# RayforceDB/rayforce

Measured on AMD Instinct MI355X. Metric: rows/s on filter→group-by→sum, 1e9-row i64/f64; % HBM roofline at 1/2/4/8 GPU, higher is better.
Workload: dtype f64

## Files before the change

rayforce_amd/csrc/rfx_group_plane.hip:

```cpp
#include "rfx_part_common.hpp"
#include <stdlib.h>

#define PL_T 1024
#define PL_WAVES (PL_T / RFX_WAVE)
#define PL_WROWS 512
#define PL_BLOCK_ROWS (1 << 18)
#define PL_DELTA_BITS 18
#define PL_SLOT_BITS 14
#define PL_QCAP 320
#define PL_QFLUSH 24
#define PL_SPIN_LIMIT (1u << 14)
#define PL_MAX_NV 3
#ifndef PL_META64_PLAIN
#define PL_META64_PLAIN 1
#endif

struct PlaneArgs {
    int nblk;
    int nv;
    unsigned pmask;
    i64 block_rows;
    unsigned c0;
    u64 *vals[PL_MAX_NV];
    unsigned *meta;
    unsigned *cnt;
    unsigned *ctl;
};
struct PlSh {
    unsigned dead, _pad[3];
    i64 red[3][PL_WAVES];
};
template <int PBITS, int VGL, bool HK>
__host__ __device__ constexpr int pl_parts() { return (HK && PBITS == 8 && VGL == 4) ? 192 : (1 << PBITS); }
template <int NV, int PBITS, int VGL, bool HK = false>
__host__ __device__ constexpr size_t pl_lds_bytes() {
    return (size_t)pl_parts<PBITS, VGL, HK>() * ((size_t)(2 << VGL) * (NV * 8 + 4) + 8 + 4) + (size_t)PL_WAVES * PL_QCAP * 4 + sizeof(PlSh) + 64;
}
typedef u64 pl_v2 __attribute__((ext_vector_type(2)));
typedef unsigned pl_m2 __attribute__((ext_vector_type(2)));
#define PL_LD(ptr) __hip_atomic_load((ptr), __ATOMIC_RELAXED, __HIP_MEMORY_SCOPE_WORKGROUP)
#define PL_ST(ptr, v) __hip_atomic_store((ptr), (v), __ATOMIC_RELAXED, __HIP_MEMORY_SCOPE_WORKGROUP)

template <int NC, int NP, int NV, int PBITS, int VGL, bool HK = false>
__global__ __launch_bounds__(PL_T) void k_plane_scatter(const Plan P, const PlaneArgs A) {
    constexpr int PARTS = pl_parts<PBITS, VGL, HK>();
    constexpr bool P192 = PARTS != (1 << PBITS);
    constexpr unsigned VG = 1u << VGL, RING = 2u << VGL;
    constexpr bool KVI = HK && NV == 2 && PBITS == 8 && VGL == 3;
    constexpr unsigned LPD = VG / 2;
    extern __shared__ __attribute__((aligned(16))) unsigned char pl_smem[];
    u64 *vring = (u64 *)pl_smem;
    unsigned *mring = (unsigned *)(vring + (size_t)NV * PARTS * RING);
    unsigned *words = mring + (size_t)PARTS * RING;
    unsigned *tail = words + PARTS * 2;
    unsigned *fq = tail + PARTS;
    PlSh &L = *(PlSh *)(fq + PL_WAVES * PL_QCAP);
    PredSet<NP> S;
    predset_load<NP>(P, S);
    const int tid = threadIdx.x, lane = tid & 63, wv = tid >> 6;
    unsigned *myq = fq + wv * PL_QCAP;
    const i64 r0 = (i64)blockIdx.x * A.block_rows;
    const i64 r1 = (r0 + A.block_rows < P.nrows) ? r0 + A.block_rows : P.nrows;
    const u64 region = ((u64)blockIdx.x * (u64)PARTS) * A.c0;
    for (int i = tid; i < PARTS; i += PL_T) {
        tail[i] = 0;
        words[2 * i] = 0;
        words[2 * i + 1] = 0;
    }
    if (tid == 0) L.dead = 0;
    __syncthreads();
    i64 mn = RFX_INF_I64_D, mx = RFX_NULL_I64_D;
    unsigned nsel = 0;
    int qn = 0;

    auto flush_queue = [&]() __attribute__((always_inline)) {
        asm volatile("" ::: "memory");
        for (int i0 = 0; i0 < qn; i0 += 64 / (int)LPD) {
            const int idx = i0 + (lane / (int)LPD);
            if (idx < qn) {
                const unsigned d = myq[idx];
                const unsigned p = d & 0xFFu, gi = (d >> 8) & 0x3FFFFFu, pl = d >> 30, sub = lane & (LPD - 1u);
                if (pl < 3) {
                    const pl_v2 x = *(const pl_v2 *)(vring + ((size_t)pl * PARTS + p) * RING + (gi & 1u) * VG + sub * 2);
                    if constexpr (KVI) {
                        __builtin_nontemporal_store(x, (pl_v2 *)(A.vals[0] + 2 * (region + (u64)p * A.c0 + (u64)gi * VG) + (u64)pl * VG + sub * 2));
                    } else {
                        u64 *dst = (NV == 1 ? A.vals[0] : (pl == 0 ? A.vals[0] : (pl == 1 ? A.vals[1] : A.vals[2])));
                        __builtin_nontemporal_store(x, (pl_v2 *)(dst + region + (u64)p * A.c0 + (u64)gi * VG + sub * 2));
                    }
                } else if (sub < LPD / 2) {
                    const pl_v2 x = *(const pl_v2 *)(mring + (size_t)p * RING + (gi & 1u) * VG + sub * 4);
                    if constexpr (KVI || (VGL == 4 && PL_META64_PLAIN)) *(pl_v2 *)(A.meta + region + (u64)p * A.c0 + (u64)gi * VG + sub * 4) = x;
                    else __builtin_nontemporal_store(x, (pl_v2 *)(A.meta + region + (u64)p * A.c0 + (u64)gi * VG + sub * 4));
                }
            }
        }
        asm volatile("" ::: "memory");
        for (int i = lane; i < qn; i += 64) {
            const unsigned d = myq[i];
            if ((d >> 30) == 3u) atomicAdd(&words[2 * (d & 0xFFu) + ((d >> 8) & 1u)], 256u - VG);
        }
        qn = 0;
    };

    auto place = [&](const bool on, const u64 key, const u64 (&val)[NV], const unsigned delta) __attribute__((always_inline)) {
        const u64 kh = HK ? rfx_hash_index_u64(RFX_U64_HASH_SEED, key) : key;
        const unsigned p = P192 ? (unsigned)(((kh >> 32) * (u64)PARTS) >> 32) : (HK ? (unsigned)(kh >> (64 - PBITS)) : ((unsigned)key & (unsigned)(PARTS - 1)));
        unsigned seq = 0;
        if (on) {
            const i64 k = (i64)key;
            mn = k < mn ? k : mn;
            mx = k > mx ? k : mx;
            seq = atomicAdd(&tail[p], 1u);
            if (seq >= A.c0) PL_ST(&L.dead, 1u);
        }
        const unsigned g = seq >> VGL;
        unsigned *w = &words[2 * p + (g & 1u)];
        bool todo = on && seq < A.c0;
        for (unsigned it = 0;; it++) {
            bool ready = false;
            if (todo) ready = (PL_LD(w) >> 8) == (g >> 1);
            bool comp = false;
            if (ready) {
                const unsigned at = p * RING + (seq & (RING - 1u));
#pragma unroll
                for (int j = 0; j < NV; j++) vring[(size_t)j * PARTS * RING + at] = val[j];
                mring[at] = ((unsigned)(P192 ? (kh >> 18) : (HK ? (kh >> (64 - PBITS - PL_SLOT_BITS)) : (key >> PBITS))) & ((1u << PL_SLOT_BITS) - 1u)) | (delta << PL_SLOT_BITS);
                asm volatile("" ::: "memory");
                comp = (atomicAdd(w, 1u) & 0xFFu) == VG - 1u;
                todo = false;
            }
            const u64 cb = __ballot(comp);
            if (cb) {
                if (comp) {
                    const unsigned at = (unsigned)qn + (unsigned)(NV + 1) * __builtin_amdgcn_mbcnt_hi((unsigned)(cb >> 32), __builtin_amdgcn_mbcnt_lo((unsigned)cb, 0u));
#pragma unroll
                    for (int j = 0; j < NV; j++) myq[at + j] = p | (g << 8) | ((unsigned)j << 30);
                    myq[at + NV] = p | (g << 8) | (3u << 30);
                }
                qn += (NV + 1) * __popcll(cb);
            }
            if (!__any(todo)) break;
            flush_queue();
            if (PL_LD(&L.dead) || it > PL_SPIN_LIMIT) {
                PL_ST(&L.dead, 1u);
                break;
            }
            if (it) __builtin_amdgcn_s_sleep(4);
        }
        if (qn >= PL_QFLUSH) flush_queue();
    };

    bool alive = true;
    auto step = [&](const u64 (&v)[NC][8], const unsigned m, const i64 sbase) __attribute__((always_inline)) {
        const unsigned dbase = (unsigned)(sbase - r0);
        const unsigned valid = m;
        if constexpr (NP == 0) {
            nsel += (unsigned)__popc(valid);
#pragma unroll
            for (int e = 0; e < 8; e++) {
                u64 val[NV];
#pragma unroll
                for (int j = 0; j < NV; j++) val[j] = v[1 + j][e];
                place((valid >> e) & 1u, v[0][e], val, dbase + (unsigned)((e >> 1) * 128 + (e & 1)));
            }
        } else {
            unsigned rem = m;
            nsel += (unsigned)__popc(rem);
            u64 t[1 + NV][8];
#pragma unroll
            for (int c = 0; c < 1 + NV; c++) {
#pragma unroll
                for (int q = 0; q < 8; q++) {
                    t[c][q] = v[c][q];
                    if constexpr (NV > 1) asm volatile("" : "+v"(t[c][q]));
                }
            }
            while (__any(rem != 0u)) {
                const bool on = rem != 0u;
                const unsigned e = (unsigned)__builtin_ctz(rem | 0x100u);
                rem &= rem - 1u;
                u64 key = t[0][0], val[NV];
#pragma unroll
                for (int j = 0; j < NV; j++) val[j] = t[1 + j][0];
#pragma unroll
                for (int q = 1; q < 8; q++) {
                    const bool is = e == (unsigned)q;
                    key = is ? t[0][q] : key;
#pragma unroll
                    for (int j = 0; j < NV; j++) val[j] = is ? t[1 + j][q] : val[j];
                }
                place(on, key, val, dbase + (e >> 1) * 128u + (e & 1u));
            }
        }
        flush_queue();
        if (PL_LD(&L.dead)) alive = false;
    };

    const i64 nsteps = (r1 - r0 + PL_WROWS - 1) / PL_WROWS;
    const i64 nfull = (r1 - r0) / PL_WROWS;
    {
        u64 va[NC][8];
        for (i64 s = wv; s < nfull && alive; s += PL_WAVES) {
            const i64 base = r0 + s * PL_WROWS + lane * 2;
            if constexpr (NP == 0) {
#pragma unroll
                for (int c = 0; c < NC; c++) {
#pragma unroll
                    for (int j = 0; j < 4; j++) {
                        const u64x2 t = rfx_ld2(P.cols[c] + base + j * 128);
                        va[c][2 * j] = t.x;
                        va[c][2 * j + 1] = t.y;
                    }
                }
                step(va, 0xffu, base);
            } else {
#pragma unroll
                for (int c = 0; c < NC; c++) {
                    if ((A.pmask >> c) & 1u) {
#pragma unroll
                        for (int j = 0; j < 4; j++) {
                            const u64x2 t = rfx_ld2(P.cols[c] + base + j * 128);
                            va[c][2 * j] = t.x;
                            va[c][2 * j + 1] = t.y;
                        }
                    } else {
#pragma unroll
                        for (int e = 0; e < 8; e++) va[c][e] = 0;
                    }
                }
                const unsigned m = eval_preds<NC, 8, NP>(S, va, 0xffu);
#pragma unroll
                for (int c = 0; c < NC; c++) {
                    if (!((A.pmask >> c) & 1u)) {
#pragma unroll
                        for (int j = 0; j < 4; j++) {
                            if ((m >> (2 * j)) & 3u) {
                                const u64x2 t = rfx_ld2(P.cols[c] + base + j * 128);
                                va[c][2 * j] = t.x;
                                va[c][2 * j + 1] = t.y;
                            }
                        }
                    }
                }
                step(va, m, base);
            }
        }
    }
    if (nfull < nsteps && (nfull % PL_WAVES) == wv && alive) {
        u64 va[NC][8];
        const i64 base = r0 + nfull * PL_WROWS + lane * 2;
        unsigned valid = 0;
#pragma unroll
        for (int e = 0; e < 8; e++) {
            const i64 row = base + (e >> 1) * 128 + (e & 1);
            const bool in = row < r1;
            valid |= (unsigned)in << e;
#pragma unroll
            for (int c = 0; c < NC; c++) va[c][e] = in ? P.cols[c][row] : 0ULL;
        }
        step(va, (NP == 0) ? valid : eval_preds<NC, 8, NP>(S, va, valid), base);
    }
    __syncthreads();
    if (L.dead) {
        if (tid == 0) atomicExch(&A.ctl[1], 1u);
        return;
    }
    for (int i = tid; i < PARTS * (NV + 1) * (int)LPD; i += PL_T) {
        const unsigned sub = (unsigned)i & (LPD - 1u), p = ((unsigned)i / LPD) % (unsigned)PARTS, pl = ((unsigned)i / LPD) / (unsigned)PARTS;
        const unsigned t = tail[p];
        if (!(t & (VG - 1u))) continue;
        const unsigned gi = t >> VGL;
        if (pl < (unsigned)NV) {
            const pl_v2 x = *(const pl_v2 *)(vring + ((size_t)pl * PARTS + p) * RING + (gi & 1u) * VG + sub * 2);
            if constexpr (KVI) {
                *(pl_v2 *)(A.vals[0] + 2 * (region + (u64)p * A.c0 + (u64)gi * VG) + (u64)pl * VG + sub * 2) = x;
            } else {
                u64 *dst = (NV == 1 ? A.vals[0] : (pl == 0 ? A.vals[0] : (pl == 1 ? A.vals[1] : A.vals[2])));
                *(pl_v2 *)(dst + region + (u64)p * A.c0 + (u64)gi * VG + sub * 2) = x;
            }
        } else if (sub < LPD / 2) {
            const pl_v2 x = *(const pl_v2 *)(mring + (size_t)p * RING + (gi & 1u) * VG + sub * 4);
            *(pl_v2 *)(A.meta + region + (u64)p * A.c0 + (u64)gi * VG + sub * 4) = x;
        }
    }
    for (int i = tid; i < PARTS; i += PL_T) A.cnt[(size_t)blockIdx.x * PARTS + i] = tail[i];
    i64 sel = (i64)nsel;
    for (int s2 = 32; s2 >= 1; s2 >>= 1) {
        const i64 omn = (i64)rfx_shfl_xor_u64((u64)mn, s2), omx = (i64)rfx_shfl_xor_u64((u64)mx, s2);
        mn = omn < mn ? omn : mn;
        mx = omx > mx ? omx : mx;
        sel += (i64)rfx_shfl_xor_u64((u64)sel, s2);
    }
    if (lane == 0) {
        L.red[0][wv] = mn;
        L.red[1][wv] = mx;
        L.red[2][wv] = sel;
    }
    __syncthreads();
    if (tid == 0) {
        for (int w2 = 1; w2 < PL_WAVES; w2++) {
            mn = L.red[0][w2] < mn ? L.red[0][w2] : mn;
            mx = L.red[1][w2] > mx ? L.red[1][w2] : mx;
            sel += L.red[2][w2];
        }
        unsigned long long *g = (unsigned long long *)A.ctl + 8;
        if (sel > 0) {
            atomicMax(&g[0], ~((unsigned long long)mn ^ 0x8000000000000000ULL));
            atomicMax(&g[1], (unsigned long long)mx ^ 0x8000000000000000ULL);
            atomicAdd(&g[2], (unsigned long long)sel);
        }
    }
}

struct PlaneAggArgs {
    i64 kmin, range;
    i64 local;
    int split;
    int excl;
    int first_read;
    int nblk, pbits;
    int agg_pl[RFX_MAX_AGGS];
    i64 block_rows;
    unsigned c0;
    const u64 *vals[PL_MAX_NV];
    const unsigned *meta;
    const unsigned *cnt;
    u64 *first;
    u64 *acc[RFX_MAX_AGGS];
    u64 *cntt[RFX_MAX_AGGS];
};
#define PL_FIRST_NONE 0xFFFFFFFFu

template <int THREADS, int NVL, bool FAST>
__global__ __launch_bounds__(THREADS) void k_plane_aggregate(const Plan P, const PlaneAggArgs A) {
    extern __shared__ __attribute__((aligned(16))) u64 pl_agg_smem[];
    const int tid = threadIdx.x;
    const int p = blockIdx.x / A.split, s = blockIdx.x % A.split;
    const i64 local = A.local;
    int kind[RFX_MAX_AGGS], f64[RFX_MAX_AGGS], skip[RFX_MAX_AGGS], cnt_of[RFX_MAX_AGGS], apl[RFX_MAX_AGGS];
    int ncnt = 0;
#pragma unroll
    for (int a = 0; a < RFX_MAX_AGGS; a++) {
        kind[a] = (a < P.nagg) ? P.aggs[a].kind : -1;
        f64[a] = (a < P.nagg) ? P.aggs[a].f64 : 0;
        skip[a] = (a < P.nagg) ? P.aggs[a].skipnull : 0;
        apl[a] = (a < P.nagg) ? A.agg_pl[a] : -1;
        cnt_of[a] = -1;
        if (kind[a] >= 0 && agg_has_cnt(kind[a], f64[a])) cnt_of[a] = ncnt++;
    }
    u64 *accs = pl_agg_smem;
    unsigned *first = (unsigned *)(accs + (i64)P.nagg * local);
    unsigned *cnts = first + local;
    for (i64 i = tid; i < local; i += THREADS) first[i] = PL_FIRST_NONE;
#pragma unroll
    for (int a = 0; a < RFX_MAX_AGGS; a++) {
        if (kind[a] < 0) continue;
        const u64 id = acc_identity(kind[a], f64[a]);
        for (i64 i = tid; i < local; i += THREADS) accs[(i64)a * local + i] = id;
        if (cnt_of[a] >= 0) {
            for (i64 i = tid; i < local; i += THREADS) cnts[(i64)cnt_of[a] * local + i] = 0u;
        }
    }
    __syncthreads();
    const unsigned shift = (unsigned)(((i64)p - A.kmin) >> A.pbits);
    auto apply = [&](unsigned mm, i64 rbase, const u64 (&x)[NVL]) __attribute__((always_inline)) {
        const unsigned mask = (1u << PL_SLOT_BITS) - 1u;
        const unsigned slot = ((mm & mask) + shift) & mask;
        if ((i64)slot >= local) return;
        const unsigned row = (unsigned)(rbase + (i64)(mm >> PL_SLOT_BITS));
        if (A.first_read) {
            if (row < first[slot]) atomicMin(&first[slot], row);
        } else __hip_atomic_fetch_min(&first[slot], row, __ATOMIC_RELAXED, __HIP_MEMORY_SCOPE_WORKGROUP);
        if constexpr (FAST) {
            unsafeAtomicAdd((double *)&accs[slot], rfx_as_f64(x[0]));
            return;
        }
#pragma unroll
        for (int a = 0; a < RFX_MAX_AGGS; a++) {
            if (kind[a] < 0) continue;
            u64 xv = 0;
#pragma unroll
            for (int j = 0; j < NVL; j++)
                if (apl[a] == j) xv = x[j];
            group_apply(&accs[(i64)a * local + slot], cnt_of[a] >= 0 ? &cnts[(i64)cnt_of[a] * local + slot] : (unsigned *)0, kind[a], f64[a], xv, skip[a]);
        }
    };
    const int lane = tid & 63;
    constexpr int NW = THREADS / 64;
    const int Q = A.split * NW;
    struct Batch {
        pl_v2 val[NVL][2];
        pl_m2 m[2];
        unsigned n, i0;
        int b;
    };
    auto load = [&](bool live, int b, unsigned i0, unsigned n, Batch &B) __attribute__((always_inline)) {
        B.b = live ? b : 0;
        B.i0 = live ? i0 : 0u;
        B.n = live ? n : 0u;
        const u64 base = (((u64)B.b << A.pbits) + (u64)p) * A.c0;
#pragma unroll
        for (int k = 0; k < 2; k++) {
            unsigned i = B.i0 + ((unsigned)k * 64u + (unsigned)lane) * 2u;
            i = i < A.c0 - 2u ? i : A.c0 - 2u;
#pragma unroll
            for (int j = 0; j < NVL; j++) B.val[j][k] = __builtin_nontemporal_load((const pl_v2 *)(A.vals[j] + base + i));
            B.m[k] = __builtin_nontemporal_load((const pl_m2 *)(A.meta + base + i));
        }
    };
    auto consume = [&](const Batch &B) __attribute__((always_inline)) {
        const i64 rbase = (i64)B.b * A.block_rows;
#pragma unroll
        for (int k = 0; k < 2; k++) {
            const unsigned i = B.i0 + ((unsigned)k * 64u + (unsigned)lane) * 2u;
            if (i < B.n) {
                u64 x[NVL];
#pragma unroll
                for (int j = 0; j < NVL; j++) x[j] = B.val[j][k].x;
                apply(B.m[k].x, rbase, x);
                if (i + 1 < B.n) {
#pragma unroll
                    for (int j = 0; j < NVL; j++) x[j] = B.val[j][k].y;
                    apply(B.m[k].y, rbase, x);
                }
            }
        }
    };
    const int q = __builtin_amdgcn_readfirstlane(s * NW + (tid >> 6));
    const int nreg = q < A.nblk ? (A.nblk - q + Q - 1) / Q : 0;
    unsigned *wcnt = cnts + (i64)ncnt * local + (tid >> 6) * 64;
    int r = -1;
    int b = q;
    unsigned i0 = 0, n = 0;
    auto advance = [&]() __attribute__((always_inline)) {
        for (;;) {
            if (r >= 0 && i0 < n) return true;
            r++;
            if (r >= nreg) return false;
            if ((r & 63) == 0) {
                const int r0 = r + lane;
                wcnt[lane] = (r0 < nreg) ? A.cnt[((size_t)(q + r0 * Q) << A.pbits) + p] : 0u;
            }
            n = (unsigned)__builtin_amdgcn_readfirstlane((int)wcnt[r & 63]);
            b = q + r * Q;
            i0 = 0;
        }
    };
    Batch B0, B1;
    bool h0 = advance();
    load(h0, b, i0, n, B0);
    i0 += 256u;
    while (h0) {
        const bool h1 = advance();
        load(h1, b, i0, n, B1);
        i0 += 256u;
        consume(B0);
        if (!h1) break;
        h0 = advance();
        load(h0, b, i0, n, B0);
        i0 += 256u;
        consume(B1);
    }
    __syncthreads();
    for (i64 i = tid; i < local; i += THREADS) {
        const unsigned f = first[i];
        if (f == PL_FIRST_NONE) continue;
        const i64 g = (i << A.pbits) | (i64)(((u64)p - (u64)A.kmin) & (u64)((1 << A.pbits) - 1));
        if (g >= A.range) continue;
        const u64 fr = (u64)P.row0 + (u64)f;
        if (A.excl) {
            if (fr < A.first[g]) A.first[g] = fr;
#pragma unroll
            for (int a = 0; a < RFX_MAX_AGGS; a++) {
                if (kind[a] < 0) continue;
                const bool hc = cnt_of[a] >= 0;
                group_merge_cell_plain(&A.acc[a][g], hc ? &A.cntt[a][g] : (u64 *)0, kind[a], f64[a], accs[(i64)a * local + i], hc ? (u64)cnts[(i64)cnt_of[a] * local + i] : 0ULL);
            }
            continue;
        }
        if (fr < A.first[g]) atomicMin((unsigned long long *)&A.first[g], (unsigned long long)fr);
#pragma unroll
        for (int a = 0; a < RFX_MAX_AGGS; a++) {
            if (kind[a] < 0) continue;
            const bool hc = cnt_of[a] >= 0;
            group_merge_cell(&A.acc[a][g], hc ? &A.cntt[a][g] : (u64 *)0, kind[a], f64[a], accs[(i64)a * local + i], hc ? (u64)cnts[(i64)cnt_of[a] * local + i] : 0ULL);
        }
    }
}

int rfx_chunk_reserve(rfx_ctx *c, size_t bytes);
static size_t pl_al256(size_t x) { return (x + 255) & ~(size_t)255; }

static void plane_layout(rfx_ctx *c, int nblk, int pbits, unsigned c0, int nv, PlaneArgs *A, size_t *total, int parts = 0) {
    const size_t regions = parts ? (size_t)nblk * (size_t)parts : (size_t)nblk << pbits;
    const size_t o_cnt = 256;
    const size_t o_meta = o_cnt + pl_al256(regions * 4), o_val = o_meta + pl_al256(regions * c0 * 4);
    const size_t plane = pl_al256(regions * c0 * 8);
    if (total) *total = o_val + plane * nv;
    char *w = (char *)c->d_chunk;
    A->nblk = nblk;
    A->nv = nv;
    A->c0 = c0;
    A->ctl = (unsigned *)w;
    A->cnt = (unsigned *)(w + o_cnt);
    A->meta = (unsigned *)(w + o_meta);
    for (int j = 0; j < nv; j++) A->vals[j] = (u64 *)(w + o_val + plane * j);
}

template <int NC, int NP, int NV, int PBITS, int VGL, bool HK = false>
static int launch_plane_scatter_inst(rfx_ctx *c, const Plan &P, const PlaneArgs &A) {
    constexpr size_t lds = pl_lds_bytes<NV, PBITS, VGL, HK>();
    static_assert(lds <= 160 * 1024, "rings beyond a CU's LDS");
    static unsigned long long attr_set = 0;
    if (!((attr_set >> (c->device & 63)) & 1ull)) {
        RFX_HIP_CHECK(hipFuncSetAttribute((const void *)k_plane_scatter<NC, NP, NV, PBITS, VGL, HK>, hipFuncAttributeMaxDynamicSharedMemorySize, (int)lds));
        __atomic_fetch_or(&attr_set, 1ull << (c->device & 63), __ATOMIC_RELAXED);
    }
    hipLaunchKernelGGL((k_plane_scatter<NC, NP, NV, PBITS, VGL, HK>), dim3(A.nblk), dim3(PL_T), lds, c->stream, P, A);
    return RFX_OK;
}
template <int NC, int NV, int PBITS, int VGL, bool HK = false>
static int launch_plane_scatter_np(rfx_ctx *c, const Plan &P, const PlaneArgs &A) {
    if (P.npred == 0) return launch_plane_scatter_inst<NC, 0, NV, PBITS, VGL, HK>(c, P, A);
    if (P.npred == 1) return launch_plane_scatter_inst<NC, 1, NV, PBITS, VGL, HK>(c, P, A);
    if (P.npred <= 3) return launch_plane_scatter_inst<NC, 3, NV, PBITS, VGL, HK>(c, P, A);
    return launch_plane_scatter_inst<NC, RFX_MAX_PREDS, NV, PBITS, VGL, HK>(c, P, A);
}
static int launch_plane_scatter(rfx_ctx *c, const Plan &P, const PlaneArgs &A, int pbits) {
    const int extra = P.ncols - 1 - A.nv;
    if (extra < 0 || extra > 2) return RFX_ESTATE;
    if (A.nv == 1) {
        if (pbits == 7) return extra == 0 ? launch_plane_scatter_np<2, 1, 7, 5>(c, P, A) : (extra == 1 ? launch_plane_scatter_np<3, 1, 7, 5>(c, P, A) : launch_plane_scatter_np<4, 1, 7, 5>(c, P, A));
        return extra == 0 ? launch_plane_scatter_np<2, 1, 8, 4>(c, P, A) : (extra == 1 ? launch_plane_scatter_np<3, 1, 8, 4>(c, P, A) : launch_plane_scatter_np<4, 1, 8, 4>(c, P, A));
    }
    if (pbits != 7 || extra > 1) return RFX_ESTATE;
    if (A.nv == 2) return extra == 0 ? launch_plane_scatter_np<3, 2, 7, 4>(c, P, A) : launch_plane_scatter_np<4, 2, 7, 4>(c, P, A);
    return extra == 0 ? launch_plane_scatter_np<4, 3, 7, 4>(c, P, A) : launch_plane_scatter_np<5, 3, 7, 4>(c, P, A);
}

static int plane_value_cols(const Plan &P, int *vcol, int *agg_plane) {
    int nv = 0;
    for (int a = 0; a < P.nagg; a++) {
        const PlanAgg &ag = P.aggs[a];
        agg_plane[a] = -1;
        if (ag.kind == RFX_AGG_COUNT || ag.kind == RFX_AGG_FIRST || ag.col < 0) continue;
        if (ag.col >= RFX_XCOL) return -1;
        int j = 0;
        for (; j < nv; j++)
            if (vcol[j] == ag.col) break;
        if (j == nv) {
            if (nv >= PL_MAX_NV) return -1;
            vcol[nv++] = ag.col;
        }
        agg_plane[a] = j;
    }
    return nv;
}
static size_t plane_agg_lds(const Plan &P, int a0, int a1, i64 local) {
    size_t cells8 = 0, cells4 = 1;
    for (int a = a0; a < a1; a++) {
        cells8++;
        if (agg_has_cnt(P.aggs[a].kind, P.aggs[a].f64)) cells4++;
    }
    return (size_t)local * (cells8 * 8 + cells4 * 4) + 16 * 64 * 4 + 64;
}
#define PL_AGG_LDS_MAX (150 * 1024)
static bool plane_agg_fits(const Plan &P, i64 local) {
    for (int a = 0; a < P.nagg; a++)
        if (plane_agg_lds(P, a, a + 1, local) > PL_AGG_LDS_MAX) return false;
    return P.nagg >= 1;
}

struct PlaneState {
    int valid, npred, logic, nblk, pbits, nv;
    unsigned c0;
    const void *key;
    const void *val[PL_MAX_NV];
    i64 nrows;
    i64 seen;
    u64 sig[RFX_MAX_PREDS][6];
};
static PlaneState *plane_state(rfx_ctx *c) {
    if (!c->ext_p[2]) c->ext_p[2] = calloc(1, sizeof(PlaneState));
    return (PlaneState *)c->ext_p[2];
}
void rfx_plane_invalidate(rfx_ctx *c) {
    if (c->ext_p[2]) ((PlaneState *)c->ext_p[2])->valid = 0;
}
void rfx_plane_release(rfx_ctx *c) {
    free(c->ext_p[2]);
    c->ext_p[2] = NULL;
}
static void plane_pred_sig(const Plan &P, u64 (*sig)[6]) {
    for (int i = 0; i < P.npred; i++) {
        const PlanPred &q = P.preds[i];
        sig[i][0] = (u64)(uintptr_t)P.cols[q.col];
        sig[i][1] = q.rhs_col >= 0 ? (u64)(uintptr_t)P.cols[q.rhs_col] : 0;
        sig[i][2] = (u64)q.op;
        sig[i][3] = (u64)(q.dom_f64 | (q.lhs_cvt << 1) | (q.rhs_cvt << 2) | (q.more << 3) | ((u64)q.tree << 4));
        sig[i][4] = q.rhs_bits;
        sig[i][5] = 0;
    }
}

int rfx_plane_scope(rfx_ctx *c, const Plan &P, int key_idx, const void *d_key, int npred, int logic, unsigned long long est_range, double frac,
                    i64 *kmin, i64 *kmax, i64 *seen) {
    PlaneState *st = plane_state(c);
    if (!st) return RFX_ESTATE;
    st->valid = 0;
    if (c->flags & RFX_TUNE_NO_PLANE) return RFX_ESTATE;
    int vcol[PL_MAX_NV], agg_plane[RFX_MAX_AGGS];
    const int nv = plane_value_cols(P, vcol, agg_plane);
    if (nv < 1 || P.nx > 0) return RFX_ESTATE;
    int pbits = 7;
    {
        static const char *force = getenv("RFX_PLANE_PBITS");
        const i64 l7 = (i64)((est_range + 127) >> 7);
        if (l7 + l7 / 16 > (1 << PL_SLOT_BITS) || !plane_agg_fits(P, l7 + l7 / 16)) pbits = 8;
        if (force && nv == 1) pbits = atoi(force) == 7 ? 7 : 8;
    }
    if (pbits == 8 && nv > 1) return RFX_ESTATE;
    const i64 est_local = (i64)((est_range + (1ULL << pbits) - 1) >> pbits);
    if (est_local > (1 << PL_SLOT_BITS) || !plane_agg_fits(P, est_local)) return RFX_ESTATE;
    const i64 nrows = P.nrows;
    const i64 nblk64 = (nrows + PL_BLOCK_ROWS - 1) / PL_BLOCK_ROWS;
    if (nblk64 > (1 << 20) || nrows >= 0xFFFFFFF0LL) return RFX_ESTATE;
    double share = (double)PL_BLOCK_ROWS / (double)(1 << pbits);
    if (npred > 0) share *= (frac * 1.3 + 0.01 < 1.0 ? frac * 1.3 + 0.01 : 1.0);
    unsigned c0 = (unsigned)(share * 1.25 + 160.0);
    c0 = (c0 + 127u) & ~127u;
    PlaneArgs A;
    memset(&A, 0, sizeof(A));
    size_t need = 0;
    plane_layout(c, (int)nblk64, pbits, c0, nv, &A, &need);
    if (rfx_chunk_reserve(c, need) != RFX_OK) return RFX_ESTATE;
    plane_layout(c, (int)nblk64, pbits, c0, nv, &A, NULL);
    A.block_rows = PL_BLOCK_ROWS;
    Plan Pc = P;
    {
        int perm[RFX_MAX_COLS + PL_MAX_NV], inv[RFX_MAX_COLS], n2 = 0;
        for (int i = 0; i < P.ncols; i++) inv[i] = -1;
        perm[n2++] = key_idx;
        inv[key_idx] = 0;
        for (int j = 0; j < nv; j++) {
            if (inv[vcol[j]] < 0) inv[vcol[j]] = n2;
            perm[n2++] = vcol[j];
        }
        for (int i = 0; i < P.ncols; i++)
            if (inv[i] < 0) {
                inv[i] = n2;
                perm[n2++] = i;
            }
        if (n2 > 1 + nv + 2 || n2 > RFX_MAX_COLS) return RFX_ESTATE;
        Pc.ncols = n2;
        for (int i = 0; i < n2; i++) Pc.cols[i] = P.cols[perm[i]];
        for (int i = 0; i < P.npred; i++) {
            Pc.preds[i].col = inv[P.preds[i].col];
            if (P.preds[i].rhs_col >= 0) Pc.preds[i].rhs_col = inv[P.preds[i].rhs_col];
        }
    }
    for (int i = 0; i < Pc.npred; i++) {
        A.pmask |= 1u << Pc.preds[i].col;
        if (Pc.preds[i].rhs_col >= 0) A.pmask |= 1u << Pc.preds[i].rhs_col;
    }
    if (getenv("RFX_PLANE_LOAD_ALL")) A.pmask = 0xFFu;
    RFX_HIP_CHECK(hipMemsetAsync(A.ctl, 0, 256, c->stream));
    c->ext_i[3 + RFX_STAT_PLANE_SCATTER]++;
    RFX_KERNEL_BEGIN(c);
    int rc = launch_plane_scatter(c, Pc, A, pbits);
    RFX_KERNEL_END(c);
    if (rc != RFX_OK) return rc;
    RFX_HIP_CHECK(hipGetLastError());
    unsigned *hctl = (unsigned *)c->h_pin;
    RFX_HIP_CHECK(hipMemcpyAsync(hctl, A.ctl, 256, hipMemcpyDeviceToHost, c->stream));
    RFX_HIP_CHECK(hipStreamSynchronize(c->stream));
    if (hctl[1]) {
        c->ext_i[3 + RFX_STAT_PLANE_FALLBACK]++;
        return RFX_ESTATE;
    }
    const u64 *hs = (const u64 *)hctl + 8;
    *seen = (i64)hs[2];
    plane_state(c)->seen = *seen;
    *kmin = (i64)(~hs[0] ^ 0x8000000000000000ULL);
    *kmax = (i64)(hs[1] ^ 0x8000000000000000ULL);
    if (*seen > 0 && *kmin == RFX_NULL_I64_D) return RFX_ESTATE;
    if (*seen == 0) return RFX_OK;
    st->valid = 1;
    st->key = d_key;
    for (int j = 0; j < nv; j++) st->val[j] = (const void *)P.cols[vcol[j]];
    st->nrows = nrows;
    st->npred = npred;
    st->logic = logic;
    st->nblk = (int)nblk64;
    st->pbits = pbits;
    st->nv = nv;
    st->c0 = c0;
    plane_pred_sig(P, st->sig);
    return RFX_OK;
}

template <int THREADS, int NVL, bool FAST>
static int launch_plane_aggregate_inst(rfx_ctx *c, const Plan &P, const PlaneAggArgs &G, int grid, size_t lds, int lds_max) {
    static unsigned long long attr_set = 0;
    if (!((attr_set >> (c->device & 63)) & 1ull)) {
        RFX_HIP_CHECK(hipFuncSetAttribute((const void *)k_plane_aggregate<THREADS, NVL, FAST>, hipFuncAttributeMaxDynamicSharedMemorySize, lds_max));
        __atomic_fetch_or(&attr_set, 1ull << (c->device & 63), __ATOMIC_RELAXED);
    }
    hipLaunchKernelGGL((k_plane_aggregate<THREADS, NVL, FAST>), dim3(grid), dim3(THREADS), lds, c->stream, P, G);
    return RFX_OK;
}
template <int THREADS>
static int launch_plane_aggregate(rfx_ctx *c, const Plan &P, const PlaneAggArgs &G, int nvl, bool fast, int grid, size_t lds, int lds_max) {
    if (nvl <= 1) return fast ? launch_plane_aggregate_inst<THREADS, 1, true>(c, P, G, grid, lds, lds_max) : launch_plane_aggregate_inst<THREADS, 1, false>(c, P, G, grid, lds, lds_max);
    if (nvl == 2) return launch_plane_aggregate_inst<THREADS, 2, false>(c, P, G, grid, lds, lds_max);
    return launch_plane_aggregate_inst<THREADS, 3, false>(c, P, G, grid, lds, lds_max);
}

int rfx_plane_accumulate(rfx_ctx *c, const Plan &P, int key_idx, const rfx_group_tables_t *t) {
    PlaneState *st = (PlaneState *)c->ext_p[2];
    if (!st || !st->valid) return RFX_ESTATE;
    int vcol[PL_MAX_NV], agg_plane[RFX_MAX_AGGS];
    bool ok = st->key == (const void *)P.cols[key_idx] && st->nrows == P.nrows && st->npred == P.npred && st->logic == P.logic && P.nx == 0;
    const int nv = ok ? plane_value_cols(P, vcol, agg_plane) : -1;
    ok = ok && nv == st->nv;
    for (int j = 0; ok && j < nv; j++) ok = st->val[j] == (const void *)P.cols[vcol[j]];
    if (ok && P.npred > 0) {
        u64 sig[RFX_MAX_PREDS][6];
        plane_pred_sig(P, sig);
        ok = memcmp(sig, st->sig, sizeof(u64) * 6 * (size_t)P.npred) == 0;
    }
    st->valid = 0;
    if (!ok || t->range <= (1 << st->pbits)) return RFX_ESTATE;
    const i64 local = (t->range + (1 << st->pbits) - 1) >> st->pbits;
    if (local > (1 << PL_SLOT_BITS) || !plane_agg_fits(P, local)) return RFX_ESTATE;
    PlaneArgs A;
    memset(&A, 0, sizeof(A));
    plane_layout(c, st->nblk, st->pbits, st->c0, st->nv, &A, NULL);
    const int nparts = 1 << st->pbits;
    RFX_KERNEL_BEGIN(c);
    int rc = RFX_OK;
    for (int a0 = 0; a0 < P.nagg && rc == RFX_OK;) {
        int a1 = a0 + 1;
        while (a1 < P.nagg && plane_agg_lds(P, a0, a1 + 1, local) <= PL_AGG_LDS_MAX) a1++;
        Plan Ps = P;
        Ps.nagg = a1 - a0;
        PlaneAggArgs G;
        memset(&G, 0, sizeof(G));
        G.kmin = t->kmin;
        G.range = t->range;
        G.local = local;
        {
            static const char *fr = getenv("RFX_PL_FIRST_READ");
            G.first_read = fr ? atoi(fr) : 1;
        }
        G.nblk = st->nblk;
        G.pbits = st->pbits;
        G.block_rows = PL_BLOCK_ROWS;
        G.c0 = st->c0;
        G.meta = A.meta;
        G.cnt = A.cnt;
        G.first = (u64 *)t->d_first;
        int used[PL_MAX_NV] = {-1, -1, -1}, nvl = 0;
        for (int a = a0; a < a1; a++) {
            Ps.aggs[a - a0] = P.aggs[a];
            G.acc[a - a0] = (u64 *)t->d_acc[a];
            G.cntt[a - a0] = (u64 *)t->d_cnt[a];
            G.agg_pl[a - a0] = -1;
            if (agg_plane[a] < 0) continue;
            int j = 0;
            for (; j < nvl; j++)
                if (used[j] == agg_plane[a]) break;
            if (j == nvl) {
                used[nvl] = agg_plane[a];
                G.vals[nvl] = A.vals[agg_plane[a]];
                nvl++;
            }
            G.agg_pl[a - a0] = j;
        }
        for (int a = a1 - a0; a < RFX_MAX_AGGS; a++) {
            Ps.aggs[a].kind = -1;
            G.agg_pl[a] = -1;
        }
        if (nvl == 0) {
            G.vals[0] = A.vals[0];
            nvl = 1;
        }
        const size_t lds = plane_agg_lds(P, a0, a1, local);
        const bool fast = Ps.nagg == 1 && Ps.aggs[0].kind == RFX_AGG_SUM && Ps.aggs[0].f64 && !Ps.aggs[0].skipnull && G.agg_pl[0] == 0;
        c->ext_i[3 + RFX_STAT_PLANE_AGGREGATE]++;
        if (lds > 52 * 1024) {
            G.split = (c->num_cus + nparts - 1) / nparts;
            if (G.split < 1) G.split = 1;
            {
                static const char *fs = getenv("RFX_PLANE_AGG_SPLIT");
                if (fs && atoi(fs) >= 1) G.split = atoi(fs);
                else if (st->seen > 0 && st->seen <= 40000000) G.split = 1;
            }
            G.excl = G.split == 1;
            rc = launch_plane_aggregate<1024>(c, Ps, G, nvl, fast, nparts * G.split, lds, 160 * 1024);
        } else {
            const int per_cu = (int)((156 * 1024) / lds) < 4 ? (int)((156 * 1024) / lds) : 4;
            G.split = (per_cu * c->num_cus + nparts - 1) / nparts;
            if (G.split < 1) G.split = 1;
            rc = launch_plane_aggregate<512>(c, Ps, G, nvl, fast, nparts * G.split, lds, 64 * 1024);
        }
        a0 = a1;
    }
    RFX_KERNEL_END(c);
    if (rc != RFX_OK) return rc;
    RFX_HIP_CHECK(hipGetLastError());
    return RFX_OK;
}

struct PlaneHashArgs {
    HashArgs H;
// ... 486 lines not shown
```

Baseline: 215.6 billion.

## Stage filtered rows in per-wave LDS buffers and drain them as full waves

For filtered (NP>0), non-hashed plane scatters, selected rows are compacted into a per-wave LDS staging buffer via ballot/mbcnt, and the buffer is drained into the partition rings once 64 records have accumulated. This replaces the old per-element serial loop over surviving lanes, so ring placement runs with full wavefronts instead of sparse, divergent masks. In exchange it adds LDS traffic for the staged records, a larger LDS footprint that may lower occupancy, and a final drain pass after the loop.

```diff
diff --git a/rayforce_amd/csrc/rfx_group_plane.hip b/rayforce_amd/csrc/rfx_group_plane.hip
--- a/rayforce_amd/csrc/rfx_group_plane.hip
+++ b/rayforce_amd/csrc/rfx_group_plane.hip
@@ -14,6 +14,11 @@
 #ifndef PL_META64_PLAIN
 #define PL_META64_PLAIN 1
 #endif
+
+#ifndef PL_STAGE
+#define PL_STAGE 1
+#endif
+#define PL_STAGE_RECS 128
 
 struct PlaneArgs {
     int nblk;
@@ -36,6 +41,12 @@
 __host__ __device__ constexpr size_t pl_lds_bytes() {
     return (size_t)pl_parts<PBITS, VGL, HK>() * ((size_t)(2 << VGL) * (NV * 8 + 4) + 8 + 4) + (size_t)PL_WAVES * PL_QCAP * 4 + sizeof(PlSh) + 64;
 }
+template <int NV>
+__host__ __device__ constexpr size_t pl_stage_bytes() { return (size_t)PL_WAVES * PL_STAGE_RECS * (NV * 8 + 8); }
+template <int NP, int NV, int PBITS, int VGL, bool HK>
+__host__ __device__ constexpr bool pl_staged() {
+    return PL_STAGE && NP > 0 && !HK && pl_lds_bytes<NV, PBITS, VGL, HK>() + pl_stage_bytes<NV>() <= 160 * 1024;
+}
 typedef u64 pl_v2 __attribute__((ext_vector_type(2)));
 typedef unsigned pl_m2 __attribute__((ext_vector_type(2)));
 #define PL_LD(ptr) __hip_atomic_load((ptr), __ATOMIC_RELAXED, __HIP_MEMORY_SCOPE_WORKGROUP)
@@ -55,6 +66,11 @@
     unsigned *tail = words + PARTS * 2;
     unsigned *fq = tail + PARTS;
     PlSh &L = *(PlSh *)(fq + PL_WAVES * PL_QCAP);
+    constexpr bool STAGED = pl_staged<NP, NV, PBITS, VGL, HK>();
+    static_assert(!STAGED || (((size_t)PARTS * ((size_t)RING * (NV * 8 + 4) + 12) + (size_t)PL_WAVES * PL_QCAP * 4 + sizeof(PlSh)) % 16 == 0), "16-byte staged records");
+    pl_v2 *st16 = (pl_v2 *)(&L + 1) + (threadIdx.x >> 6) * PL_STAGE_RECS;
+    u64 *st8 = (u64 *)((pl_v2 *)(&L + 1) + PL_WAVES * PL_STAGE_RECS) + (size_t)(threadIdx.x >> 6) * (NV - 1) * PL_STAGE_RECS;
+    unsigned nst = 0;
     PredSet<NP> S;
     predset_load<NP>(P, S);
     const int tid = threadIdx.x, lane = tid & 63, wv = tid >> 6;
@@ -103,14 +119,9 @@
         qn = 0;
     };
 
-    auto place = [&](const bool on, const u64 key, const u64 (&val)[NV], const unsigned delta) __attribute__((always_inline)) {
-        const u64 kh = HK ? rfx_hash_index_u64(RFX_U64_HASH_SEED, key) : key;
-        const unsigned p = P192 ? (unsigned)(((kh >> 32) * (u64)PARTS) >> 32) : (HK ? (unsigned)(kh >> (64 - PBITS)) : ((unsigned)key & (unsigned)(PARTS - 1)));
+    auto place_at = [&](const bool on, const unsigned p, const unsigned mw, const u64 (&val)[NV]) __attribute__((always_inline)) {
         unsigned seq = 0;
         if (on) {
-            const i64 k = (i64)key;
-            mn = k < mn ? k : mn;
-            mx = k > mx ? k : mx;
             seq = atomicAdd(&tail[p], 1u);
             if (seq >= A.c0) PL_ST(&L.dead, 1u);
         }
@@ -125,7 +136,7 @@
                 const unsigned at = p * RING + (seq & (RING - 1u));
 #pragma unroll
                 for (int j = 0; j < NV; j++) vring[(size_t)j * PARTS * RING + at] = val[j];
-                mring[at] = ((unsigned)(P192 ? (kh >> 18) : (HK ? (kh >> (64 - PBITS - PL_SLOT_BITS)) : (key >> PBITS))) & ((1u << PL_SLOT_BITS) - 1u)) | (delta << PL_SLOT_BITS);
+                mring[at] = mw;
                 asm volatile("" ::: "memory");
                 comp = (atomicAdd(w, 1u) & 0xFFu) == VG - 1u;
                 todo = false;
@@ -149,6 +160,39 @@
             if (it) __builtin_amdgcn_s_sleep(4);
         }
         if (qn >= PL_QFLUSH) flush_queue();
+    };
+    auto route = [&](const bool on, const u64 key, const unsigned delta, unsigned &p, unsigned &mw) __attribute__((always_inline)) {
+        const u64 kh = HK ? rfx_hash_index_u64(RFX_U64_HASH_SEED, key) : key;
+        p = P192 ? (unsigned)(((kh >> 32) * (u64)PARTS) >> 32) : (HK ? (unsigned)(kh >> (64 - PBITS)) : ((unsigned)key & (unsigned)(PARTS - 1)));
+        mw = ((unsigned)(P192 ? (kh >> 18) : (HK ? (kh >> (64 - PBITS - PL_SLOT_BITS)) : (key >> PBITS))) & ((1u << PL_SLOT_BITS) - 1u)) | (delta << PL_SLOT_BITS);
+        if (on) {
+            const i64 k = (i64)key;
+            mn = k < mn ? k : mn;
+            mx = k > mx ? k : mx;
+        }
+    };
+    auto place = [&](const bool on, const u64 key, const u64 (&val)[NV], const unsigned delta) __attribute__((always_inline)) {
+        unsigned p, mw;
+        route(on, key, delta, p, mw);
+        place_at(on, p, mw, val);
+    };
+    auto drain = [&]() __attribute__((always_inline)) {
+        const unsigned base = nst > 64u ? nst - 64u : 0u;
+        const bool on = (unsigned)lane < nst - base;
+        unsigned p = 0, mw = 0;
+        u64 val[NV];
+#pragma unroll
+        for (int j = 0; j < NV; j++) val[j] = 0;
+        if (on) {
+            const pl_v2 r = st16[base + lane];
+            mw = (unsigned)r.x;
+            p = (unsigned)(r.x >> 32);
+            val[0] = r.y;
+#pragma unroll
+            for (int j = 1; j < NV; j++) val[j] = st8[(j - 1) * PL_STAGE_RECS + base + lane];
+        }
+        nst = base;
+        place_at(on, p, mw, val);
     };
 
     bool alive = true;
@@ -163,6 +207,28 @@
 #pragma unroll
                 for (int j = 0; j < NV; j++) val[j] = v[1 + j][e];
                 place((valid >> e) & 1u, v[0][e], val, dbase + (unsigned)((e >> 1) * 128 + (e & 1)));
+            }
+        } else if constexpr (STAGED) {
+            nsel += (unsigned)__popc(m);
+#pragma unroll
+            for (int e = 0; e < 8; e++) {
+                const bool on = (m >> e) & 1u;
+                const u64 b = __ballot(on);
+                if (b) {
+                    if (on) {
+                        unsigned p, mw;
+                        route(true, v[0][e], dbase + (unsigned)((e >> 1) * 128 + (e & 1)), p, mw);
+                        const unsigned at = nst + __builtin_amdgcn_mbcnt_hi((unsigned)(b >> 32), __builtin_amdgcn_mbcnt_lo((unsigned)b, 0u));
+                        pl_v2 r;
+                        r.x = ((u64)p << 32) | mw;
+                        r.y = v[1][e];
+                        st16[at] = r;
+#pragma unroll
+                        for (int j = 1; j < NV; j++) st8[(j - 1) * PL_STAGE_RECS + at] = v[1 + j][e];
+                    }
+                    nst += (unsigned)__popcll(b);
+                    if (nst >= 64u) drain();
+                }
             }
         } else {
             unsigned rem = m;
@@ -260,6 +326,12 @@
             for (int c = 0; c < NC; c++) va[c][e] = in ? P.cols[c][row] : 0ULL;
         }
         step(va, (NP == 0) ? valid : eval_preds<NC, 8, NP>(S, va, valid), base);
+    }
+    if constexpr (STAGED) {
+        if (nst && alive) {
+            drain();
+            flush_queue();
+        }
     }
     __syncthreads();
     if (L.dead) {
@@ -510,8 +582,8 @@
 
 template <int NC, int NP, int NV, int PBITS, int VGL, bool HK = false>
 static int launch_plane_scatter_inst(rfx_ctx *c, const Plan &P, const PlaneArgs &A) {
-    constexpr size_t lds = pl_lds_bytes<NV, PBITS, VGL, HK>();
-    static_assert(lds <= 160 * 1024, "rings beyond a CU's LDS");
+    constexpr size_t lds = pl_lds_bytes<NV, PBITS, VGL, HK>() + (pl_staged<NP, NV, PBITS, VGL, HK>() ? pl_stage_bytes<NV>() : 0);
+    static_assert(lds <= 160 * 1024, "rings (and the staging area) beyond a CU's LDS");
     static unsigned long long attr_set = 0;
     if (!((attr_set >> (c->device & 63)) & 1ull)) {
         RFX_HIP_CHECK(hipFuncSetAttribute((const void *)k_plane_scatter<NC, NP, NV, PBITS, VGL, HK>, hipFuncAttributeMaxDynamicSharedMemorySize, (int)lds));
```

After: 217.3 billion, median of 6. About the same (+0.8%).
